# ahcorde/visualSLAM_Android

Measured on AMD Instinct MI355X. Metric: frames/sec (TrackFrame+local BA) on 640×480 synthetic, 1/2/4/8 GPU, higher is better.
Workload: dtype f64

## Files before the change

### visualslam_android_amd/csrc/track.hip

```cpp
#include "vslam_internal.h"
#include "patch_dev.h"
#include "pvs_perm.h"

#define TRK_THREADS 256
#define SORT_CAP 4096
static_assert(SORT_CAP == PVS_SORT_CAP, "a level's list (at most max_points entries) fits the permutation's sort buffer");

template <class T>
DEVFN bool td_project(T& td, int& flags, const double* pos, const Pose& pose, const CamModel& cam, CamProj& pr) {
  flags &= ~TDF_IN_IMAGE;
  double c[3];
  pose_xform(pose, pos, c);
  td.cam[0] = c[0]; td.cam[1] = c[1]; td.cam[2] = c[2];
  if (c[2] < 0.001) return false;
  const double implane[2] = {c[0] / c[2], c[1] / c[2]};
  if (implane[0] * implane[0] + implane[1] * implane[1] > cam.largest_radius * cam.largest_radius) return false;
  pr = cam_project(cam, implane[0], implane[1]);
  td.image[0] = pr.im[0]; td.image[1] = pr.im[1];
  if (pr.invalid) return true;
  if (td.image[0] < 0 || td.image[1] < 0 || td.image[0] > cam.size[0] || td.image[1] > cam.size[1]) return true;
  flags |= TDF_IN_IMAGE;
  return true;
}

// ... 116 lines not shown
  for (int l = 0; l < NLEV; l++) pvs_shuffle_list(pvs_sortbuf(), pvs + l * P, cnt[l], h, l);
}

template <bool SHUFFLE>
__global__ __launch_bounds__(TRK_THREADS) void k_plan(MapDev m, TrackParams tp, int stage) {
  const int s = blockIdx.x;
  TrackerState* st = &m.st[s];
  if (!trk_runs_track_map(st)) return;
  const int P = tp.max_points;
  TrackData* td = m.td + (size_t)s * P;
  const MapPointDev* pts = m.pts + (size_t)s * P;
  int* pvs = m.pvs_list + (size_t)s * NLEV * P;
  int2* slist = m.search_list + (size_t)s * P;
  int* ilist = m.iter_list + (size_t)s * P;
  const int lane = threadIdx.x & 63, wave = threadIdx.x >> 6;
  __shared__ int cnt[NLEV];
  __shared__ int wcnt[TRK_THREADS / 64][NLEV];
  __shared__ int plan[4];
  if (stage == 0) {
    if (threadIdx.x < NLEV) cnt[threadIdx.x] = 0;
    __syncthreads();
    const int n = st->n_points;
    constexpr int PLAN_CH = 16;
    for (int base = 0; base < n; base += PLAN_CH * TRK_THREADS) {
      const int first = base + threadIdx.x * PLAN_CH;
      int lv[PLAN_CH], c[NLEV] = {0, 0, 0, 0};
#pragma unroll
      for (int k = 0; k < PLAN_CH; k++) { const int i = first + k; lv[k] = m.pt_level[(size_t)s * P + (i < n ? i : n - 1)]; if (i >= n) lv[k] = -1; }
#pragma unroll
      for (int k = 0; k < PLAN_CH; k++)
#pragma unroll
        for (int l = 0; l < NLEV; l++) c[l] += lv[k] == l;
      int off[NLEV];
#pragma unroll
      for (int l = 0; l < NLEV; l++) {
        int inc = c[l];
        for (int d = 1; d < 64; d <<= 1) { const int t = __shfl_up(inc, d); if (lane >= d) inc += t; }
        if (lane == 63) wcnt[wave][l] = inc;
        off[l] = inc - c[l];
      }
      __syncthreads();
#pragma unroll
      for (int l = 0; l < NLEV; l++) { off[l] += cnt[l]; for (int w = 0; w < wave; w++) off[l] += wcnt[w][l]; }
#pragma unroll
      for (int k = 0; k < PLAN_CH; k++) {
#pragma unroll
        for (int l = 0; l < NLEV; l++) if (lv[k] == l) pvs[l * P + off[l]++] = first + k;
      }
      __syncthreads();
      if (threadIdx.x < NLEV) { int t = cnt[threadIdx.x]; for (int w = 0; w < TRK_THREADS / 64; w++) t += wcnt[w][threadIdx.x]; cnt[threadIdx.x] = t; }
      __syncthreads();
    }
    if constexpr (SHUFFLE) {
      const unsigned seed = st->pvs_seed;
      if (seed) pvs_shuffle_levels(pvs, P, cnt, seed, st->frame);
    }
    if (threadIdx.x == 0) {
      for (int l = 0; l < NLEV; l++) { st->pvs_count[l] = cnt[l]; st->pvs_head[l] = 0; }
      unsigned nCoarseMax = tp.coarse_max, nCoarseRange = tp.coarse_range;
      st->did_coarse = 0;
      bool bTry = true;
      if (tp.coarse_disabled || st->msd_vel < tp.coarse_min_vel || nCoarseMax == 0) bTry = false;
      if (st->just_recovered) { bTry = true; nCoarseMax *= 2; nCoarseRange *= 2; st->just_recovered = 0; }
      int c3 = 0, c2 = 0;
      const unsigned n3 = cnt[3], n2 = cnt[2];
      if (bTry && n3 + n2 > (unsigned)tp.coarse_min) {
        unsigned take3 = n3 <= nCoarseMax ? n3 : nCoarseMax;
        st->pvs_head[3] = take3;
        c3 = take3;
        if (take3 < nCoarseMax) {
          const unsigned more = nCoarseMax - take3;
          if (n2 <= more) { c3 = 0; c2 = n2; st->pvs_head[2] = n2; }
          else { c2 = more; st->pvs_head[2] = more; }
        }
      }
      plan[0] = c3; plan[1] = c2;
      st->coarse_range = nCoarseRange;
      st->n_coarse = c3 + c2; st->n_search = c3 + c2; st->n_iter = c3 + c2;
    }
    __syncthreads();
    const int c3 = plan[0], c2 = plan[1];
    for (int e = threadIdx.x; e < c3 + c2; e += TRK_THREADS) {
      const int idx = e < c3 ? pvs[3 * P + e] : pvs[2 * P + (e - c3)];
      slist[e] = make_int2(idx, tp.coarse_subpix_its);
      ilist[e] = idx;
    }
  } else {
    __shared__ Pose pose;
    if (threadIdx.x == 0) {
      pose = st->pose_cur;
      const int nit = st->n_iter;
      const int h3 = st->pvs_head[3], n3 = st->pvs_count[3] - h3;
      int nother = (st->pvs_count[2] - st->pvs_head[2]) + st->pvs_count[1] + st->pvs_count[0];
      int nFine = tp.max_patches - (nit + n3);
      if (nFine < 0) nFine = 0;
      if constexpr (SHUFFLE) *pvs_chopped() = nother > nFine && nFine > 0 && st->pvs_seed != 0;
      if (nother > nFine) nother = nFine;
      plan[0] = nit; plan[1] = n3; plan[2] = nother;
      st->fine_range = st->did_coarse ? 5 : 10;
      st->n_l3 = n3; st->n_search = n3 + nother; st->n_iter = nit + n3 + nother;
    }
    __syncthreads();
    const int nit = plan[0], n3 = plan[1], nother = plan[2];
    const int h3 = st->pvs_head[3], h2 = st->pvs_head[2];
    const int r2 = st->pvs_count[2] - h2, r1 = st->pvs_count[1];
    const int did_coarse = st->did_coarse;
    const uint64_t* rest_order = nullptr;
    if constexpr (SHUFFLE) {
      uint64_t* sortbuf = pvs_sortbuf();
      if (*pvs_chopped()) {
        const int nrest = r2 + r1 + st->pvs_count[0];
        pvs_block_fill<TRK_THREADS>(sortbuf, nrest, pvs_frame_hash(st->pvs_seed, st->frame), PVS_LIST_REST, nullptr);
        pvs_block_sort<TRK_THREADS>(sortbuf, nrest);
        rest_order = sortbuf;
      }
    }
    for (int e = threadIdx.x; e < n3 + nother; e += TRK_THREADS) {
      int idx, its;
      if (e < n3) { idx = pvs[3 * P + h3 + e]; its = tp.fine_subpix_its; }
      else {
        int k = e - n3;
        if constexpr (SHUFFLE) if (rest_order) k = (int)(uint32_t)rest_order[k];
        if (k < r2) idx = pvs[2 * P + h2 + k];
        else if (k < r2 + r1) idx = pvs[1 * P + (k - r2)];
        else idx = pvs[0 * P + (k - r2 - r1)];
        its = 0;
      }
      if (e < n3 || did_coarse) td_project_and_derivs(td[idx], m.pt_flags[(size_t)s * P + idx], pts[idx].pos, pose, tp.cam);
      slist[e] = make_int2(idx, its);
      ilist[nit + e] = idx;
    }
  }
}

struct SearchArgs {
  const uint8_t* img[NLEV]; size_t img_sstride[NLEV]; int img_pitch[NLEV];
  const uint32_t* corners[NLEV]; const int* rowlut[NLEV]; const int* ncorners;
  int w[NLEV], h[NLEV], cap[NLEV];
  size_t kf_stride[NLEV];
  int kf_pitch[NLEV];
  int nblk, S;
};


#define TRK_XCDS 8
DEVFN void xcd_stream_block(int nblk, int S, int& s, int& blk) {
  const int i = blockIdx.x, x = i % TRK_XCDS, j = i / TRK_XCDS;
  blk = j % nblk;
  s = (j / nblk) * TRK_XCDS + x;
  if (s >= S) s = -1;
}
static int xcd_grid(int nblk, int S) { return nblk * ((S + TRK_XCDS - 1) / TRK_XCDS) * TRK_XCDS; }

template <int PS, int G>
__global__ __launch_bounds__(64) void k_searchN(MapDev m, TrackParams tp, SearchArgs a, int stage) {
  constexpr int NPIX = PS * PS, HALF = PS / 2, PPW = 64 / G;
  int s, bx;
  xcd_stream_block(a.nblk, a.S, s, bx);
  if (s < 0) return;
  TrackerState* st = &m.st[s];
  if (!trk_runs_track_map(st)) return;
  const int nsearch = st->n_search;
  if (bx * PPW >= nsearch) return;
  const int lane = threadIdx.x, grp = lane / G, sub = lane % G;
  const bool rowact = sub < PS;
  const int e = bx * PPW + grp;
  bool act = e < nsearch;
  const bool lead = sub == 0;
  const int2 ent = act ? m.search_list[(size_t)s * tp.max_points + e] : make_int2(0, 0);
  const int idx = ent.x, nSubPixIts = ent.y;
  const int nRangeL0 = stage == 0 ? st->coarse_range : st->fine_range;
  TrackData& td = m.td[(size_t)s * tp.max_points + idx];
  int& tdlevel = m.pt_level[(size_t)s * tp.max_points + idx];
  int& tdflags = m.pt_flags[(size_t)s * tp.max_points + idx];
  const MapPointDev& p = m.pts[(size_t)s * tp.max_points + idx];
  uint8_t* gtmpl = m.tmpl + ((size_t)s * tp.max_points + idx) * TMPL_PITCH;
  const int level = act ? tdlevel : 0, scale = 1 << level;
  int flags = tdflags;

  double m2[4];
  template_warp_matrix(td.warp_inv, scale, m2);
  const bool refresh = (!(flags & TDF_HAVE_LAST) || warp_moved(m2, td.last_warp)) && act;
  PRow<PS> trow = zero_row<PS>();
  if (rowact) trow = load_row<PS>(gtmpl + sub * PS);
  const int tsum_cached = td.tsum, tsumsq_cached = td.tsumsq;
  int tsum, tsumsq;
  if (__any(refresh)) {
    const int sl = p.src_level;
    const uint8_t* src = m.kf_img[sl] + ((size_t)s * tp.max_keyframes + p.src_kf) * a.kf_stride[sl];
    const int sp = a.kf_pitch[sl], iw = a.w[sl], ih = a.h[sl];
    const TemplateWarp tw = template_warp<PS>(m2, p.irx, p.iry, iw, ih);
    double px = tw.x0, py = tw.y0;
#pragma unroll 1
    for (int i = 0; i < PS - 1; i++) {
      if (i < sub) warp_row_step<PS>(tw, px, py);
    }
    if (refresh) {
      int nOutside = 0, sum = 0, sumsq = 0;
      if (rowact) {
        trow = zero_row<PS>();
#pragma unroll
        for (int j = 0; j < PS; j++) {
          const int v = warp_sample(tw, src, sp, px, py, nOutside);
          warp_pixel_step(tw, px, py);
          trow.w[j >> 2] |= (unsigned)v << (8 * (j & 3));
          sum += v; sumsq += v * v;
        }
        __builtin_memcpy(gtmpl + sub * PS, &trow, PS);
      }
      nOutside = grp_sum<G>(nOutside);
      tsum = grp_sum<G>(sum); tsumsq = grp_sum<G>(sumsq);
      flags = nOutside ? (flags | TDF_TMPL_BAD) : (flags & ~TDF_TMPL_BAD);
      flags |= TDF_HAVE_LAST;
      if (lead) { td.tsum = tsum; td.tsumsq = tsumsq; for (int i = 0; i < 4; i++) td.last_warp[i] = m2[i]; }
    }
  }
  if (!refresh) { tsum = tsum_cached; tsumsq = tsumsq_cached; }
  if (act && (flags & TDF_TMPL_BAD)) {
    if (lead) tdflags = flags & ~(TDF_IN_IMAGE | TDF_FOUND);
    act = false;
  }
  for (int l = 0; l < NLEV; l++) {
    const int c = __popcll(__ballot(act && lead && level == l));
    if (lane == 0 && c) atomicAdd(&st->attempted[l], c);
  }

  const double irx = td.image[0] / scale, iry = td.image[1] / scale;
  const int rows = a.h[level], cols = a.w[level];
  const CoarseWindow cw = coarse_window(irx, iry, nRangeL0, scale, rows);
  int nBestSSD = tp.max_ssd + 1;
  uint32_t bestCorner = 0;
  unsigned nEval = 0;
  const uint32_t* corners = a.corners[level] + (size_t)s * a.cap[level];
  const uint8_t* img = a.img[level] + (size_t)s * a.img_sstride[level];
  const int ip = a.img_pitch[level];
  int i0 = 0, i1 = 0;
  if (act && !cw.empty) {
    const int* lut = a.rowlut[level] + (size_t)s * (rows + 1);
    i0 = lut[cw.top];
    i1 = cw.bottom_plus_one >= rows ? a.ncorners[s * NLEV + level] : lut[cw.bottom_plus_one];
  }
  const double r2max = (double)(cw.range * cw.range);
  constexpr int CPL = 4;
  for (int base = i0; __any(base < i1); base += CPL * G) {
    uint32_t cval[CPL];
    unsigned long long gm = 0;
#pragma unroll
    for (int j = 0; j < CPL; j++) {
      const int ci = base + j * G + sub;
      cval[j] = ci < i1 ? corners[ci] : 0u;
    }
#pragma unroll
    for (int j = 0; j < CPL; j++) {
      const int ci = base + j * G + sub;
      bool ok = false;
      if (ci < i1) {
        const int cx = cval[j] & 0xFFFF, cy = cval[j] >> 16;
        if (!(cx < cw.left || cx > cw.right)) {
          const double dx = irx - cx, dy = iry - cy;
          ok = !(dx * dx + dy * dy > r2max);
        }
      }
      gm |= (unsigned long long)((unsigned)(__ballot(ok) >> (grp * G)) & ((1u << G) - 1u)) << (j * G);
    }
    nEval += __popcll(gm);
    while (__any(gm != 0)) {
      int kk[2]; bool has[2], inside[2]; uint32_t c[2]; PRow<PS> n[2];
#pragma unroll
      for (int u = 0; u < 2; u++) {
        has[u] = gm != 0;
        kk[u] = has[u] ? __ffsll((long long)gm) - 1 : 0;
        gm &= gm - 1;
        const int j = kk[u] / G;
        const uint32_t csel = j == 0 ? cval[0] : (j == 1 ? cval[1] : (j == 2 ? cval[2] : cval[3]));
        c[u] = __shfl(csel, grp * G + (kk[u] % G));
        const int cx = c[u] & 0xFFFF, cy = c[u] >> 16;
        inside[u] = has[u] && cx >= HALF && cy >= HALF && cx < cols - HALF && cy < rows - HALF;
        n[u] = zero_row<PS>();
        if (inside[u] && rowact) n[u] = load_row<PS>(img + (size_t)(cy - HALF + sub) * ip + (cx - HALF));
      }
#pragma unroll
      for (int u = 0; u < 2; u++) {
        int sA, sQ, sX;
        grp_zmssd_sums<PS, G>(n[u], trow, sA, sQ, sX);
        if (has[u]) {
          const int ssd = inside[u] ? zmssd_score<NPIX>(tsum, tsumsq, sA, sQ, sX) : tp.max_ssd + 1;
          if (ssd < nBestSSD) { nBestSSD = ssd; bestCorner = c[u]; }
        }
      }
    }
  }
  flags |= TDF_SEARCHED;
  {
    const int tot = wave_sum(act && lead ? (int)nEval : 0);
    if (lane == 0 && tot) atomicAdd(&st->n_zmssd, (unsigned long long)tot);
  }
  bool found = act && nBestSSD < tp.max_ssd;
  if (act && !found && lead) tdflags = flags & ~TDF_FOUND;
  const uint32_t bc = found ? bestCorner : 0u;
  const double coarse[2] = {level_zero_pos((double)(bc & 0xFFFF), level), level_zero_pos((double)(bc >> 16), level)};
  if (found) flags |= TDF_FOUND;
  const bool dosub = found && nSubPixIts > 0;
  if (found) {
    flags = dosub ? (flags | TDF_SUBPIX) : (flags & ~TDF_SUBPIX);
    if (lead) { tdflags = flags; td.sqrt_inv_noise = 1.0 / scale; td.vfound[0] = coarse[0]; td.vfound[1] = coarse[1]; }
  }
  for (int l = 0; l < NLEV; l++) {
    const int c = __popcll(__ballot(found && !dosub && lead && level == l));
    if (lane == 0 && c) atomicAdd(&st->found[l], c);
  }
}

template <int PS, int G>
DEVFN void subpix_block(const MapDev& m, const TrackParams& tp, const SearchArgs& a, TrackerState* st, int s, int nsub, int blk) {
  constexpr int HALF = PS / 2, PPW = 64 / G, NW = (PS + 3) / 4, Q = PS - 2;
  const int lane = threadIdx.x, grp = lane / G, sub = lane % G;
  const int e = blk * PPW + grp;
  const bool lead = sub == 0;
  const int2 ent = e < nsub ? m.search_list[(size_t)s * tp.max_points + e] : make_int2(0, 0);
  const int idx = ent.x, nSubPixIts = ent.y;
  TrackData& td = m.td[(size_t)s * tp.max_points + idx];
  int& tdlevel = m.pt_level[(size_t)s * tp.max_points + idx];
  int& tdflags = m.pt_flags[(size_t)s * tp.max_points + idx];
  int flags = tdflags;
  const bool dosub = e < nsub && nSubPixIts > 0 && (flags & TDF_FOUND) && (flags & TDF_SUBPIX);
  if (!__any(dosub)) return;
  const int level = dosub ? tdlevel : 0, scale = 1 << level;
  const int rows = a.h[level], cols = a.w[level];
  const uint8_t* img = a.img[level] + (size_t)s * a.img_sstride[level];
  const int ip = a.img_pitch[level];
  PRow<PS> trow = zero_row<PS>(), rup, rdn;
  if (sub < PS) trow = load_row<PS>(m.tmpl + ((size_t)s * tp.max_points + idx) * TMPL_PITCH + sub * PS);
  const bool rowok = sub >= 1 && sub <= Q;
#pragma unroll
  for (int k = 0; k < NW; k++) { rup.w[k] = __shfl(trow.w[k], lane - 1); rdn.w[k] = __shfl(trow.w[k], lane + 1); }
  double gx[Q], gy[Q];
  double h00 = 0, h01 = 0, h02 = 0, h11 = 0, h12 = 0, h22 = 0;
#pragma unroll
  for (int x = 1; x <= Q; x++) {
    gx[x - 1] = 0; gy[x - 1] = 0;
    if (rowok) {
      gx[x - 1] = 0.5 * (row_byte(trow, x + 1) - row_byte(trow, x - 1));
      gy[x - 1] = 0.5 * (row_byte(rdn, x) - row_byte(rup, x));
      h00 += gx[x - 1] * gx[x - 1]; h01 += gx[x - 1] * gy[x - 1]; h02 += gx[x - 1];
      h11 += gy[x - 1] * gy[x - 1]; h12 += gy[x - 1]; h22 += 1.0;
    }
  }
  h00 = grp_sum<G>(h00); h01 = grp_sum<G>(h01); h02 = grp_sum<G>(h02);
  h11 = grp_sum<G>(h11); h12 = grp_sum<G>(h12); h22 = grp_sum<G>(h22);
  const double H[9] = {h00, h01, h02, h01, h11, h12, h02, h12, h22};
  double Hinv[9];
  inv3(H, Hinv);
  double sub0 = td.vfound[0], sub1 = td.vfound[1], meanDiff = 0.0;
  bool running = dosub, converged = false;
  for (int it = 0; __any(running); it++) {
    if (it >= nSubPixIts) running = false;
    double cx = 0, cy = 0;
    if (running) {
      cx = level_n_pos(sub0, level); cy = level_n_pos(sub1, level);
      const int xb = (int)(cx > 0.0 ? cx + 0.5 : cx - 0.5), yb = (int)(cy > 0.0 ? cy + 0.5 : cy - 0.5);
      const int b = HALF + 1;
      if (!(xb >= b && yb >= b && xb < cols - b && yb < rows - b)) running = false;
    }
    double p0[Q], p1[Q], p2[Q];
#pragma unroll
    for (int x = 0; x < Q; x++) { p0[x] = 0; p1[x] = 0; p2[x] = 0; }
    if (running && rowok) {
      const double bx = cx - HALF, by = cy - HALF;
      const double dX = bx - floor(bx), dY = by - floor(by);
      const float fTL = (float)((1.0 - dX) * (1.0 - dY)), fTR = (float)((dX) * (1.0 - dY));
      const float fBL = (float)((1.0 - dX) * (dY)), fBR = (float)((dX) * (dY));
      const uint8_t* r0 = img + (size_t)((int)by + sub) * ip + (int)bx + 1;
      const PRow<PS> q0 = load_row<PS>(r0), q1 = load_row<PS>(r0 + ip);
#pragma unroll
      for (int x = 1; x <= Q; x++) {
        const float fPixel = fTL * row_byte(q0, x - 1) + fTR * row_byte(q0, x) + fBL * row_byte(q1, x - 1) + fBR * row_byte(q1, x);
        const double dDiff = (fPixel - (float)row_byte(trow, x)) + meanDiff;
        p0[x - 1] = dDiff * gx[x - 1]; p1[x - 1] = dDiff * gy[x - 1]; p2[x - 1] = dDiff;
      }
    }
    double a0 = 0, a1 = 0, a2 = 0;
#pragma unroll 1
    for (int y = 1; y <= Q; y++) {
      if (sub == y) {
#pragma unroll
        for (int x = 0; x < Q; x++) { a0 += p0[x]; a1 += p1[x]; a2 += p2[x]; }
      }
      const int src = grp * G + y;
      a0 = __shfl(a0, src); a1 = __shfl(a1, src); a2 = __shfl(a2, src);
    }
    if (running) {
      const double u0 = Hinv[0] * a0 + Hinv[1] * a1 + Hinv[2] * a2;
      const double u1 = Hinv[3] * a0 + Hinv[4] * a1 + Hinv[5] * a2;
      const double u2 = Hinv[6] * a0 + Hinv[7] * a1 + Hinv[8] * a2;
      sub0 -= u0 * scale; sub1 -= u1 * scale; meanDiff -= u2;
      if (u0 * u0 + u1 * u1 < 0.03 * 0.03) { converged = true; running = false; }
    }
  }
  if (dosub && lead) {
    if (!converged) tdflags = flags & ~TDF_FOUND;
    else { td.vfound[0] = sub0; td.vfound[1] = sub1; }
  }
  for (int l = 0; l < NLEV; l++) {
    const int c = __popcll(__ballot(dosub && converged && lead && level == l));
    if (lane == 0 && c) atomicAdd(&st->found[l], c);
  }
}

#define SUBPIX_GRID 16
template <int PS, int G>
__global__ __launch_bounds__(64) void k_subpixN(MapDev m, TrackParams tp, SearchArgs a, int stage) {
  int s, bx;
  xcd_stream_block(a.nblk, a.S, s, bx);
  if (s < 0) return;
  TrackerState* st = &m.st[s];
  if (!trk_runs_track_map(st)) return;
  const int nsub = stage == 0 ? st->n_search : st->n_l3;
  for (int blk = bx; blk * (64 / G) < nsub; blk += a.nblk) subpix_block<PS, G>(m, tp, a, st, s, nsub, blk);
}

#define POSE_THREADS 128
#ifdef VSLAM_BA_PROF
__device__ unsigned long long g_pose_prof[16];
#define POSE_STAMP(id) do { if (blockIdx.x == 0 && threadIdx.x == 0) { const unsigned long long t_ = clock64(); g_pose_prof[id] += t_ - g_pose_prof[15]; g_pose_prof[15] = t_; } } while (0)
#else
#define POSE_STAMP(id) do { } while (0)
#endif
#define POSE_WAVES (POSE_THREADS / 64)
#ifndef POSE_ILP
#define POSE_ILP 2
#endif

struct PoseItem {
  double cam[3], image[2], derivs[4], vfound[2], sqrt_inv_noise;
  int flags, idx;
};
struct PoseWs { double* d; int* i; int P; };

DEVFN void item_load(PoseItem& it, const PoseWs& w, int e) {
  it.flags = w.i[e]; it.idx = w.i[w.P + e];
#pragma unroll
  for (int i = 0; i < 3; i++) it.cam[i] = w.d[(0 + i) * w.P + e];
#pragma unroll
  for (int i = 0; i < 2; i++) { it.image[i] = w.d[(3 + i) * w.P + e]; it.vfound[i] = w.d[(9 + i) * w.P + e]; }
#pragma unroll
  for (int i = 0; i < 4; i++) it.derivs[i] = w.d[(5 + i) * w.P + e];
  it.sqrt_inv_noise = w.d[11 * w.P + e];
}
DEVFN void item_store(const PoseItem& it, const PoseWs& w, int e, bool all) {
#pragma unroll
  for (int i = 0; i < 2; i++) w.d[(3 + i) * w.P + e] = it.image[i];
  if (!all) return;
  w.i[e] = it.flags;
#pragma unroll
  for (int i = 0; i < 3; i++) w.d[(0 + i) * w.P + e] = it.cam[i];
#pragma unroll
  for (int i = 0; i < 4; i++) w.d[(5 + i) * w.P + e] = it.derivs[i];
}

#define POSE_CHUNK 32
#define POSE_ENT 27
#define POSE_GRP 8
static_assert(2 * 2 * POSE_CHUNK * POSE_ENT + 2 * POSE_GRP * POSE_ENT + 64 <= SORT_CAP, "two record buffers (and the chain's two groups of read-ahead) in the sort buffer");
// ... 251 lines not shown
    const bool nonlinear = stage == 0 || iter == 0 || iter == 4 || iter == 9;
    for (int e0 = threadIdx.x; e0 < nf; e0 += POSE_ILP * POSE_THREADS) {
      PoseItem t[POSE_ILP]; double pos[POSE_ILP][3];
#pragma unroll
      for (int u = 0; u < POSE_ILP; u++) {
        const int e = e0 + u * POSE_THREADS;
        item_load(t[u], ws, e < nf ? e : nf - 1);
      }
      if (nonlinear && iter != 0) {
#pragma unroll
        for (int u = 0; u < POSE_ILP; u++)
#pragma unroll
          for (int k = 0; k < 3; k++) pos[u][k] = pts[t[u].idx].pos[k];
      }
#pragma unroll
      for (int u = 0; u < POSE_ILP; u++) {
        const int e = e0 + u * POSE_THREADS;
        if (e >= nf) continue;
        if (iter != 0) {
          if (nonlinear) td_project_and_derivs(t[u], t[u].flags, pos[u], pose, tp.cam);
          else {
            double jac[12], a = 0, b = 0;
            td_calc_jacobian(t[u], jac);
#pragma unroll
            for (int k = 0; k < 6; k++) { a += jac[k] * last_up[k]; b += jac[6 + k] * last_up[k]; }
            t[u].image[0] += a; t[u].image[1] += b;
          }
          item_store(t[u], ws, e, nonlinear);
        }
        const double r0 = (t[u].vfound[0] - t[u].image[0]) * t[u].sqrt_inv_noise;
        const double r1 = (t[u].vfound[1] - t[u].image[1]) * t[u].sqrt_inv_noise;
        sortbuf[e] = r0 * r0 + r1 * r1;
      }
    }
    __syncthreads();
    POSE_STAMP(1);
    const double override_sigma = iter > 5 ? (stage == 0 ? 1.0 : 16.0) : 0.0;
    calc_pose_update(ws, pts, nf, tp, override_sigma, stage == 1 && iter == 9, sortbuf, red, up, hist, sel);
    if (threadIdx.x == 0) pose = pose_mul(se3_exp(up), pose);
    if (threadIdx.x < 6) last_up[threadIdx.x] = up[threadIdx.x];
    __syncthreads();
    POSE_STAMP(7);
  }
  POSE_STAMP(8);
  MeasDev* cm = m.cur_meas + (size_t)s * P;
  if (stage != 0) {
    for (int i = threadIdx.x; i < st->n_points; i += POSE_THREADS) cm[i].valid = 0;
    __syncthreads();
  }
  for (int e0 = threadIdx.x; e0 < nf; e0 += POSE_GB * POSE_THREADS) {
    int idx[POSE_GB], fl[POSE_GB], lv[POSE_GB]; double v[POSE_GB][11];
#pragma unroll
    for (int u = 0; u < POSE_GB; u++) {
      const int e = e0 + u * POSE_THREADS, ec = e < nf ? e : nf - 1;
      idx[u] = ws.i[P + ec]; fl[u] = ws.i[ec];
#pragma unroll
      for (int c = 0; c < 11; c++) v[u][c] = ws.d[c * P + ec];
    }
    if (stage != 0) {
#pragma unroll
      for (int u = 0; u < POSE_GB; u++) lv[u] = m.pt_level[(size_t)s * P + idx[u]];
    }
#pragma unroll
    for (int u = 0; u < POSE_GB; u++) {
      const int e = e0 + u * POSE_THREADS;
      if (e >= nf) continue;
      TrackData& t = td[idx[u]];
      m.pt_flags[(size_t)s * P + idx[u]] = fl[u];
      for (int i = 0; i < 3; i++) t.cam[i] = v[u][i];
      for (int i = 0; i < 2; i++) t.image[i] = v[u][3 + i];
      for (int i = 0; i < 4; i++) t.derivs[i] = v[u][5 + i];
      if (stage != 0) {
        MeasDev mm;
        mm.root[0] = v[u][9]; mm.root[1] = v[u][10];
        mm.valid = 1; mm.level = (signed char)lv[u]; mm.subpix = (fl[u] & TDF_SUBPIX) ? 1 : 0; mm.source = 0 ; mm.pad = 0;
        cm[idx[u]] = mm;
        sortbuf[e] = v[u][2];
      }
    }
  }
  if (stage == 0) {
    if (threadIdx.x == 0) { st->pose_cur = pose; st->did_coarse = 1; }
    return;
  }
  __syncthreads();
  if (threadIdx.x < 2) {
    double a = 0.0;
    const bool sq = threadIdx.x == 1;
    int k = 0;
    for (; k + 8 <= nf; k += 8) {
      double z[8];
#pragma unroll
      for (int u = 0; u < 8; u++) z[u] = sortbuf[k + u];
#pragma unroll
      for (int u = 0; u < 8; u++) a += sq ? z[u] * z[u] : z[u];
    }
    for (; k < nf; k++) { const double z = sortbuf[k]; a += sq ? z * z : z; }
    red[threadIdx.x] = a;
  }
  __syncthreads();
  if (threadIdx.x != 0) return;
  const double dSum = red[0], dSumSq = red[1];
  const int nNum = nf;
  if (nNum > 20) {
    st->depth_mean = dSum / nNum;
    st->depth_sigma = sqrt((dSumSq / nNum) - (st->depth_mean) * (st->depth_mean));
  }
  st->pose_cur = pose; st->pose_final = pose;
  const bool recovered = st->recovered_now != 0;
  st->recovered_now = 0;
  if (!recovered) {
    const Pose nfo = pose_mul(pose, pose_inverse(st->start_pose));
    double motion[6];
    se3_ln(nfo, motion);
    double ss = 0;
    for (int i = 0; i < 6; i++) {
      st->velocity[i] = 0.9 * (0.5 * motion[i] + 0.5 * st->velocity[i]);
      double v = st->velocity[i];
      if (i < 3) v *= 1.0 / st->depth_mean;
      ss += v * v;
    }
    st->msd_vel = sqrt(ss);
  }
  const Pose* kfp = m.kf_pose + (size_t)s * tp.max_keyframes;
  double closest = 9999999999.9;
  for (int k = 0; k < st->n_kf; k++) { const double d = kf_linear_dist(pose, kfp[k]); if (d < closest) closest = d; }
  {
    int ta = 0, tf = 0, la = 0, lf = 0;
    for (int i = 0; i < NLEV; i++) { ta += st->attempted[i]; tf += st->found[i]; if (i >= 2) { la += st->attempted[i]; lf += st->found[i]; } }
    int quality;
    if (tf == 0 || ta == 0) quality = 0;
    else {
      const double dTotal = (double)tf / ta;
      const double dLarge = la > 10 ? (double)lf / la : dTotal;
      if (dTotal > 0.3) quality = 2; else if (dLarge < 0.13) quality = 0; else quality = 1;
    }
    if (quality == 1 && closest > tp.wiggle_scale * 10.0) quality = 0;
    if (quality == 0) st->lost_frames++; else st->lost_frames = 0;
    st->quality = quality;
  }
  if (!recovered) {
    double dDist = closest;
    dDist *= (1.0 / st->depth_mean);
    const bool need = dDist > tp.max_kf_dist_wiggle_mult * st->wiggle_depth_norm;
    if (st->quality == 2 && need && st->frame - st->last_kf_dropped > tp.min_frames_between_kf && st->n_kf < tp.max_keyframes) {
      st->kf_pending = 1;
      st->last_kf_dropped = st->frame;
    }
  }
  POSE_STAMP(9);
}

#ifdef VSLAM_BA_PROF
extern "C" int vslam_debug_pose_prof(unsigned long long* out16, int reset) {
  HIPCHK(hipDeviceSynchronize());
  HIPCHK(hipMemcpyFromSymbol(out16, HIP_SYMBOL(g_pose_prof), sizeof(unsigned long long) * 16));
  if (reset) { unsigned long long z[16] = {0}; HIPCHK(hipMemcpyToSymbol(HIP_SYMBOL(g_pose_prof), z, sizeof(z))); }
  return VSLAM_OK;
}
#endif

#define TALLOC(ptr, count) do { int _r = dev_alloc(sys, &(ptr), (count)); if (_r) return _r; } while (0)

int trk_alloc(vslam_system* sys) {
  const vslam_params& p = sys->p;
  const size_t S = sys->S, P = p.max_points, K = p.max_keyframes;
  if (P > SORT_CAP) { vslam_set_error("max_points %d exceeds %d", (int)P, SORT_CAP); return VSLAM_E_INVALID; }
  MapDev& m = sys->map;
  TALLOC(m.pts, S * P); TALLOC(m.td, S * P); TALLOC(m.tmpl, S * P * TMPL_PITCH);
  TALLOC(m.kf_meas, S * K * P); TALLOC(m.cur_meas, S * P);
  TALLOC(m.kf_pose, S * K); TALLOC(m.kf_fixed, S * K); TALLOC(m.kf_depth, S * K * 2);
  for (int l = 0; l < NLEV; l++) TALLOC(m.kf_img[l], S * K * (size_t)sys->geom[l].pitch * sys->geom[l].h);
  TALLOC(m.st, S); TALLOC(m.pvs_list, S * NLEV * P); TALLOC(m.search_list, S * P); TALLOC(m.iter_list, S * P); TALLOC(m.pt_level, S * P); TALLOC(m.pt_flags, S * P);
  TALLOC(m.pose_ws, S * POSE_WS_COMPS * P); TALLOC(m.pose_wsi, S * 2 * P);
  trk_fill_params(p, sys->tp);
  return VSLAM_OK;
}

void cam_fill(CamModel& c, const double cam5[5], double width, double height, int quirks) {
  c.size[0] = width; c.size[1] = height;
  c.focal[0] = c.size[0] * cam5[0]; c.focal[1] = c.size[1] * cam5[1];
  c.center[0] = c.size[0] * cam5[2] - 0.5; c.center[1] = c.size[1] * cam5[3] - 0.5;
  c.w = cam5[4];
  double one_over_2tan = 0;
  if (c.w != 0.0) { c.two_tan = 2.0 * vlm::vtan(c.w / 2.0); one_over_2tan = 1.0 / c.two_tan; c.winv = 1.0 / c.w; c.distortion_enabled = 1.0; }
  else { c.winv = 0; c.two_tan = 0; c.distortion_enabled = 0; }
  double v2[2];
  if (quirks & VSLAM_Q_CAM_INT_RADIUS) {
    int m1 = (int)cam5[2], m2 = (int)(1.0 - cam5[2]);
    v2[0] = (m1 > m2 ? m1 : m2) / cam5[0];
    m1 = (int)cam5[3]; m2 = (int)(1.0 - cam5[3]);
    v2[1] = (m1 > m2 ? m1 : m2) / cam5[1];
  } else {
    v2[0] = (cam5[2] > 1.0 - cam5[2] ? cam5[2] : 1.0 - cam5[2]) / cam5[0];
    v2[1] = (cam5[3] > 1.0 - cam5[3] ? cam5[3] : 1.0 - cam5[3]) / cam5[1];
  }
  const double rr = sqrt(v2[0] * v2[0] + v2[1] * v2[1]);
  c.largest_radius = c.w == 0.0 ? rr : vlm::vtan(rr * c.w) * one_over_2tan;
  c.max_r = 1.5 * c.largest_radius;
}

void trk_fill_params(const vslam_params& p, TrackParams& t) {
  cam_fill(t.cam, p.cam, p.width, p.height, p.quirks);
  t.P = p.patch_size; t.max_ssd = 500 * p.patch_size * p.patch_size;
  t.max_patches = p.max_patches_per_frame; t.coarse_min = p.coarse_min; t.coarse_max = p.coarse_max; t.coarse_range = p.coarse_range;
  t.coarse_subpix_its = p.coarse_subpix_its; t.coarse_disabled = p.coarse_disabled; t.fine_subpix_its = p.fine_subpix_its;
  t.coarse_min_vel = p.coarse_min_vel; t.wls_prior = p.wls_prior;
  t.min_frames_between_kf = p.min_frames_between_kf; t.max_kf_dist_wiggle_mult = p.max_kf_dist_wiggle_mult; t.wiggle_scale = p.wiggle_scale;
  t.ba_max_iterations = p.ba_max_iterations; t.ba_convergence_limit = p.ba_convergence_limit;
  t.ba_min_sigma2 = p.ba_min_tukey_sigma * p.ba_min_tukey_sigma; t.ba_window = p.ba_window; t.ba_min_keyframes = p.ba_min_keyframes;
  t.quirks = p.quirks; t.max_points = p.max_points; t.max_keyframes = p.max_keyframes; t.ba_delay = p.ba_delay_frames;
  t.ba_batch = p.ba_batch_frames > 1 ? p.ba_batch_frames : 1;
  t.ba_sum_order = p.ba_sum_order ? 1 : 0;
  t.grow_map = p.grow_map;
  t.idle = p.idle_iterations != 0; t.fq_cap = 8192;
  {
    double a[2], b[2];
    cam_unproject(t.cam, t.cam.size[0] / 2, t.cam.size[1] / 2, a);
    cam_unproject(t.cam, t.cam.size[0] / 2 + 1, t.cam.size[1] / 2 + 1, b);
    const double d0 = a[0] - b[0], d1 = a[1] - b[1];
    t.one_pixel_dist = sqrt(d0 * d0 + d1 * d1) / sqrt(2.0);
  }
  const int kcap_max[NLEV] = {16384, 8192, 4096, 2048};
  for (int l = 0; l < NLEV; l++) t.kcap[l] = p.max_corners[l] < kcap_max[l] ? p.max_corners[l] : kcap_max[l];

}

static void trk_search_args(vslam_system* sys, SearchArgs& a) {
  for (int l = 0; l < NLEV; l++) {
    a.img[l] = sys->fr.img[l]; a.img_sstride[l] = sys->fr.img_sstride[l]; a.img_pitch[l] = sys->fr.img_pitch[l];
    a.corners[l] = sys->fr.corners[l]; a.rowlut[l] = sys->fr.rowlut[l];
    a.w[l] = sys->geom[l].w; a.h[l] = sys->geom[l].h; a.cap[l] = sys->geom[l].cap;
    a.kf_pitch[l] = sys->geom[l].pitch; a.kf_stride[l] = (size_t)sys->geom[l].pitch * sys->geom[l].h;
  }
  a.ncorners = sys->fr.ncorners;
}

typedef void (*PlanKernel)(MapDev, TrackParams, int);
static PlanKernel plan_kernel(const vslam_system* sys) { return sys->p.pvs_shuffle_seed ? k_plan<true> : k_plan<false>; }

int trk_search_stage(vslam_system* sys, int stage) {
  const int S = sys->S, P = sys->p.max_points;
  MapDev& m = sys->map;
  const TrackParams& tp = sys->tp;
  SearchArgs a;
  trk_search_args(sys, a);
  a.S = S; a.nblk = 1;
  if (stage == 0) {
    prof_mark(sys, PROF_PVS);
    hipLaunchKernelGGL(k_motion, dim3((S + 63) / 64), dim3(64), 0, sys->stream, m, S, sys->p.use_sbi ? (const double*)sys->fr.sbi_rot : (const double*)nullptr);
    hipLaunchKernelGGL(k_pvs, dim3((P + TRK_THREADS - 1) / TRK_THREADS, S), dim3(TRK_THREADS), 0, sys->stream, m, tp);
    prof_mark(sys, PROF_PLAN_COARSE);
    hipLaunchKernelGGL(plan_kernel(sys), dim3(S), dim3(TRK_THREADS), 0, sys->stream, m, tp, 0);
    prof_mark(sys, PROF_SEARCH_COARSE);
    if (!tp.coarse_disabled || sys->p.relocalise) {
      const int nc = 2 * tp.coarse_max;
      if (tp.P == 8) {
        a.nblk = (nc + 7) / 8; hipLaunchKernelGGL((k_searchN<8, 8>), dim3(xcd_grid(a.nblk, S)), dim3(64), 0, sys->stream, m, tp, a, 0);
        if (tp.coarse_subpix_its > 0) { a.nblk = SUBPIX_GRID; hipLaunchKernelGGL((k_subpixN<8, 8>), dim3(xcd_grid(a.nblk, S)), dim3(64), 0, sys->stream, m, tp, a, 0); }
      } else {
        a.nblk = (nc + 3) / 4; hipLaunchKernelGGL((k_searchN<11, 16>), dim3(xcd_grid(a.nblk, S)), dim3(64), 0, sys->stream, m, tp, a, 0);
        if (tp.coarse_subpix_its > 0) { a.nblk = SUBPIX_GRID; hipLaunchKernelGGL((k_subpixN<11, 16>), dim3(xcd_grid(a.nblk, S)), dim3(64), 0, sys->stream, m, tp, a, 0); }
      }
    }
    prof_mark(sys, PROF_POSE_COARSE);
  } else {
    const int maxSearch = tp.max_patches + 2 * tp.coarse_max < P ? tp.max_patches + 2 * tp.coarse_max : P;
    prof_mark(sys, PROF_PLAN_FINE);
    hipLaunchKernelGGL(plan_kernel(sys), dim3(S), dim3(TRK_THREADS), 0, sys->stream, m, tp, 1);
    prof_mark(sys, PROF_SEARCH_FINE);
    if (tp.P == 8) {
      a.nblk = (maxSearch + 7) / 8; hipLaunchKernelGGL((k_searchN<8, 8>), dim3(xcd_grid(a.nblk, S)), dim3(64), 0, sys->stream, m, tp, a, 1);
      if (tp.fine_subpix_its > 0) { a.nblk = SUBPIX_GRID; hipLaunchKernelGGL((k_subpixN<8, 8>), dim3(xcd_grid(a.nblk, S)), dim3(64), 0, sys->stream, m, tp, a, 1); }
    } else {
      a.nblk = (maxSearch + 3) / 4; hipLaunchKernelGGL((k_searchN<11, 16>), dim3(xcd_grid(a.nblk, S)), dim3(64), 0, sys->stream, m, tp, a, 1);
      if (tp.fine_subpix_its > 0) { a.nblk = SUBPIX_GRID; hipLaunchKernelGGL((k_subpixN<11, 16>), dim3(xcd_grid(a.nblk, S)), dim3(64), 0, sys->stream, m, tp, a, 1); }
    }
    prof_mark(sys, PROF_POSE_FINE);
  }
  HIPCHK(hipGetLastError());
  return VSLAM_OK;
}

int trk_pose_stage(vslam_system* sys, int stage) {
  if (stage == 0 && sys->tp.coarse_disabled && !sys->p.relocalise) return VSLAM_OK;
  hipLaunchKernelGGL(k_pose, dim3(sys->S), dim3(POSE_THREADS), 0, sys->stream, sys->map, sys->tp, stage);
  HIPCHK(hipGetLastError());
  return VSLAM_OK;
}

int trk_track_map(vslam_system* sys) {
  int r = trk_search_stage(sys, 0);
  if (!r) r = trk_pose_stage(sys, 0);
  if (!r) r = trk_search_stage(sys, 1);
  if (!r) r = trk_pose_stage(sys, 1);
  return r;
}

__global__ void k_set_pvs_seed(MapDev m, int S, int stream, unsigned seed) {
  const int s = blockIdx.x * blockDim.x + threadIdx.x;
  if (s >= S || (stream >= 0 && s != stream)) return;
  m.st[s].pvs_seed = seed;
}

extern "C" int vslam_set_pvs_seed(vslam_system* sys, int stream, unsigned seed) {
  if (!sys || stream >= sys->S) { vslam_set_error("set_pvs_seed: bad argument"); return VSLAM_E_INVALID; }
// ... 50 lines not shown
```

Measured before the change: 481,300.

## Widen corner-search batches, stage candidates in LDS, process K candidates per trip

```diff
diff --git a/visualslam_android_amd/csrc/track.hip b/visualslam_android_amd/csrc/track.hip
--- a/visualslam_android_amd/csrc/track.hip
+++ b/visualslam_android_amd/csrc/track.hip
@@ -292,6 +292,48 @@
 }
 static int xcd_grid(int nblk, int S) { return nblk * ((S + TRK_XCDS - 1) / TRK_XCDS) * TRK_XCDS; }
 
+#ifndef SEARCH_N
+#define SEARCH_N 128
+#endif
+#ifndef SEARCH_K
+#define SEARCH_K 4
+#endif
+#ifdef VSLAM_BA_PROF
+#define SEARCH_PROF_SLOTS 64
+__device__ unsigned long long g_search_prof[2][SEARCH_PROF_SLOTS];
+enum { SP_ENTRY, SP_TEMPLATE, SP_LUT, SP_FILTER, SP_ZMSSD, SP_WRITE, SP_PHASES };
+#define SEARCH_PROF(...) __VA_ARGS__
+#define SEARCH_PROF_BEGIN() const bool sp_on = (blockIdx.x / TRK_XCDS) % 7 == 0; unsigned long long sp_ph[SP_PHASES] = {0, 0, 0, 0, 0, 0}, sp_t0 = clock64(); \
+  int sp_ftrips = 0, sp_ztrips = 0, sp_ncorners = 0; bool sp_refresh = false
+#define SEARCH_STAMP(id) do { if (sp_on) { const unsigned long long t_ = clock64(); sp_ph[id] += t_ - sp_t0; sp_t0 = t_; } } while (0)
+#define SEARCH_PROF_END() do { if (sp_on) search_prof_flush(g_search_prof[stage], sp_ph, sp_ftrips, sp_ztrips, sp_refresh, e < nsearch && lead, sp_ncorners, (int)nEval); } while (0)
+DEVFN void search_prof_flush(unsigned long long* g, const unsigned long long* ph, int ftrips, int ztrips, bool refresh, bool patch, int ncorners, int nsurv) {
+  if (threadIdx.x == 0) {
+    for (int i = 0; i < SP_PHASES; i++) atomicAdd(&g[i], ph[i]);
+    atomicAdd(&g[6], 1ull); atomicAdd(&g[7], refresh ? 1ull : 0ull); atomicAdd(&g[8], (unsigned long long)ftrips); atomicAdd(&g[9], (unsigned long long)ztrips);
+    atomicAdd(&g[34 + (ftrips < 5 ? ftrips : 5)], 1ull); atomicAdd(&g[40 + (ztrips < 9 ? ztrips : 9)], 1ull);
+  }
+  if (patch) {
+    atomicAdd(&g[10], (unsigned long long)((nsurv + SEARCH_K - 1) / SEARCH_K)); atomicAdd(&g[11], 1ull);
+    atomicAdd(&g[12], (unsigned long long)nsurv); atomicAdd(&g[13], (unsigned long long)ncorners);
+    const int cb = ncorners == 0 ? 0 : ncorners <= 64 ? 1 + (ncorners - 1) / 16 : ncorners <= 128 ? 5 + (ncorners - 65) / 32 : 7;
+    const int sb = nsurv <= 4 ? nsurv : nsurv <= 16 ? 5 + (nsurv - 5) / 4 : 8;
+    atomicAdd(&g[16 + cb], 1ull); atomicAdd(&g[24 + sb], 1ull);
+  }
+}
+#else
+#define SEARCH_PROF(...)
+#define SEARCH_PROF_BEGIN() do { } while (0)
+#define SEARCH_STAMP(id) do { } while (0)
+#define SEARCH_PROF_END() do { } while (0)
+#endif
+
+DEVFN void wave_lds_sync() {
+  __builtin_amdgcn_fence(__ATOMIC_RELEASE, "wavefront");
+  __builtin_amdgcn_wave_barrier();
+  __builtin_amdgcn_fence(__ATOMIC_ACQUIRE, "wavefront");
+}
+
 template <int PS, int G>
 __global__ __launch_bounds__(64) void k_searchN(MapDev m, TrackParams tp, SearchArgs a, int stage) {
   constexpr int NPIX = PS * PS, HALF = PS / 2, PPW = 64 / G;
@@ -307,6 +349,7 @@
   const int e = bx * PPW + grp;
   bool act = e < nsearch;
   const bool lead = sub == 0;
+  SEARCH_PROF_BEGIN();
   const int2 ent = act ? m.search_list[(size_t)s * tp.max_points + e] : make_int2(0, 0);
   const int idx = ent.x, nSubPixIts = ent.y;
   const int nRangeL0 = stage == 0 ? st->coarse_range : st->fine_range;
@@ -317,14 +360,22 @@
   uint8_t* gtmpl = m.tmpl + ((size_t)s * tp.max_points + idx) * TMPL_PITCH;
   const int level = act ? tdlevel : 0, scale = 1 << level;
   int flags = tdflags;
-
-  double m2[4];
-  template_warp_matrix(td.warp_inv, scale, m2);
-  const bool refresh = (!(flags & TDF_HAVE_LAST) || warp_moved(m2, td.last_warp)) && act;
+  const double td_image[2] = {td.image[0], td.image[1]};
+  const double td_warp_inv[4] = {td.warp_inv[0], td.warp_inv[1], td.warp_inv[2], td.warp_inv[3]};
+  const double td_last_warp[4] = {td.last_warp[0], td.last_warp[1], td.last_warp[2], td.last_warp[3]};
+  const int tsum_cached = td.tsum, tsumsq_cached = td.tsumsq;
   PRow<PS> trow = zero_row<PS>();
   if (rowact) trow = load_row<PS>(gtmpl + sub * PS);
-  const int tsum_cached = td.tsum, tsumsq_cached = td.tsumsq;
+    struct PatchRec { double irx, iry; int left, right; unsigned range; int flags, level, subpix_its, idx, pad; };
+  __shared__ PatchRec wrec[PPW];
+  if (lead) { wrec[grp].irx = td_image[0] / scale; wrec[grp].iry = td_image[1] / scale; }
+  SEARCH_STAMP(SP_ENTRY);
+
+  double m2[4];
+  template_warp_matrix(td_warp_inv, scale, m2);
+  const bool refresh = (!(flags & TDF_HAVE_LAST) || warp_moved(m2, td_last_warp)) && act;
   int tsum, tsumsq;
+  SEARCH_PROF(sp_refresh = __any(refresh) != 0;)
   if (__any(refresh)) {
     const int sl = p.src_level;
     const uint8_t* src = m.kf_img[sl] + ((size_t)s * tp.max_keyframes + p.src_kf) * a.kf_stride[sl];
@@ -360,67 +411,95 @@
     if (lead) tdflags = flags & ~(TDF_IN_IMAGE | TDF_FOUND);
     act = false;
   }
-  for (int l = 0; l < NLEV; l++) {
-    const int c = __popcll(__ballot(act && lead && level == l));
-    if (lane == 0 && c) atomicAdd(&st->attempted[l], c);
-  }
-
-  const double irx = td.image[0] / scale, iry = td.image[1] / scale;
+  const bool attempted = act;
+  SEARCH_STAMP(SP_TEMPLATE);
+
+  wave_lds_sync();
+  const double irx = wrec[grp].irx, iry = wrec[grp].iry;
   const int rows = a.h[level], cols = a.w[level];
   const CoarseWindow cw = coarse_window(irx, iry, nRangeL0, scale, rows);
+  int i0 = 0, i1 = 0;
+  if (act && !cw.empty) {
+    const int* lut = a.rowlut[level] + (size_t)s * (rows + 1);
+    const int below = cw.bottom_plus_one >= rows ? rows : cw.bottom_plus_one;
+    const int n_all = a.ncorners[s * NLEV + level], lut_top = lut[cw.top], lut_below = lut[below];
+    i0 = lut_top;
+    i1 = cw.bottom_plus_one >= rows ? n_all : lut_below;
+  }
   int nBestSSD = tp.max_ssd + 1;
   uint32_t bestCorner = 0;
   unsigned nEval = 0;
   const uint32_t* corners = a.corners[level] + (size_t)s * a.cap[level];
   const uint8_t* img = a.img[level] + (size_t)s * a.img_sstride[level];
   const int ip = a.img_pitch[level];
-  int i0 = 0, i1 = 0;
-  if (act && !cw.empty) {
-    const int* lut = a.rowlut[level] + (size_t)s * (rows + 1);
-    i0 = lut[cw.top];
-    i1 = cw.bottom_plus_one >= rows ? a.ncorners[s * NLEV + level] : lut[cw.bottom_plus_one];
-  }
-  const double r2max = (double)(cw.range * cw.range);
-  constexpr int CPL = 4;
+  SEARCH_PROF(sp_ncorners = i1 - i0;)
+  constexpr int CPL = SEARCH_N / G < 4 ? 4 : SEARCH_N / G, K = SEARCH_K, NM = (CPL * G + 63) / 64;
+  static_assert(64 % G == 0, "a lane group's bits of one ballot lie in one mask word");
+  constexpr int CSTRIDE = CPL * G + G;
+  __shared__ uint32_t ctrip[PPW * CSTRIDE];
+  uint32_t* const gtrip = ctrip + grp * CSTRIDE;
+  if (lead) {
+    wrec[grp].left = cw.left; wrec[grp].right = cw.right; wrec[grp].range = cw.range;
+    wrec[grp].flags = flags; wrec[grp].level = level; wrec[grp].subpix_its = nSubPixIts; wrec[grp].idx = idx;
+  }
+  wave_lds_sync();
   for (int base = i0; __any(base < i1); base += CPL * G) {
     uint32_t cval[CPL];
-    unsigned long long gm = 0;
+    unsigned long long gm[NM];
+#pragma unroll
+    for (int w = 0; w < NM; w++) gm[w] = 0;
+    const double wx = wrec[grp].irx, wy = wrec[grp].iry, r2max = (double)(wrec[grp].range * wrec[grp].range);
+    const int wleft = wrec[grp].left, wright = wrec[grp].right;
 #pragma unroll
     for (int j = 0; j < CPL; j++) {
       const int ci = base + j * G + sub;
       cval[j] = ci < i1 ? corners[ci] : 0u;
     }
+    SEARCH_STAMP(SP_LUT);
 #pragma unroll
     for (int j = 0; j < CPL; j++) {
       const int ci = base + j * G + sub;
       bool ok = false;
       if (ci < i1) {
         const int cx = cval[j] & 0xFFFF, cy = cval[j] >> 16;
-        if (!(cx < cw.left || cx > cw.right)) {
-          const double dx = irx - cx, dy = iry - cy;
+        if (!(cx < wleft || cx > wright)) {
+          const double dx = wx - cx, dy = wy - cy;
           ok = !(dx * dx + dy * dy > r2max);
         }
       }
-      gm |= (unsigned long long)((unsigned)(__ballot(ok) >> (grp * G)) & ((1u << G) - 1u)) << (j * G);
-    }
-    nEval += __popcll(gm);
-    while (__any(gm != 0)) {
-      int kk[2]; bool has[2], inside[2]; uint32_t c[2]; PRow<PS> n[2];
-#pragma unroll
-      for (int u = 0; u < 2; u++) {
-        has[u] = gm != 0;
-        kk[u] = has[u] ? __ffsll((long long)gm) - 1 : 0;
-        gm &= gm - 1;
-        const int j = kk[u] / G;
-        const uint32_t csel = j == 0 ? cval[0] : (j == 1 ? cval[1] : (j == 2 ? cval[2] : cval[3]));
-        c[u] = __shfl(csel, grp * G + (kk[u] % G));
+      gm[j * G / 64] |= (unsigned long long)((unsigned)(__ballot(ok) >> (grp * G)) & ((1u << G) - 1u)) << (j * G % 64);
+      gtrip[j * G + sub] = cval[j];
+    }
+    wave_lds_sync();
+    unsigned long long left = 0;
+#pragma unroll
+    for (int w = 0; w < NM; w++) { nEval += __popcll(gm[w]); left |= gm[w]; }
+    SEARCH_PROF(sp_ftrips++;)
+    SEARCH_STAMP(SP_FILTER);
+    while (__any(left != 0)) {
+      bool has[K], inside[K]; uint32_t c[K]; PRow<PS> n[K];
+#pragma unroll
+      for (int u = 0; u < K; u++) {
+        has[u] = left != 0;
+        int kk = 0;
+        bool taken = false;
+        left = 0;
+#pragma unroll
+        for (int w = 0; w < NM; w++) {
+          const bool here = !taken && gm[w] != 0;
+          if (here) { kk = 64 * w + __ffsll((long long)gm[w]) - 1; gm[w] &= gm[w] - 1; }
+          taken = taken || here;
+          left |= gm[w];
+        }
+        c[u] = gtrip[kk];
         const int cx = c[u] & 0xFFFF, cy = c[u] >> 16;
         inside[u] = has[u] && cx >= HALF && cy >= HALF && cx < cols - HALF && cy < rows - HALF;
         n[u] = zero_row<PS>();
         if (inside[u] && rowact) n[u] = load_row<PS>(img + (size_t)(cy - HALF + sub) * ip + (cx - HALF));
       }
 #pragma unroll
-      for (int u = 0; u < 2; u++) {
+      for (int u = 0; u < K; u++) {
+        if (u >= 2 && !__any(has[u])) break;
         int sA, sQ, sX;
         grp_zmssd_sums<PS, G>(n[u], trow, sA, sQ, sX);
         if (has[u]) {
@@ -428,27 +507,37 @@
           if (ssd < nBestSSD) { nBestSSD = ssd; bestCorner = c[u]; }
         }
       }
-    }
-  }
-  flags |= TDF_SEARCHED;
+      SEARCH_PROF(sp_ztrips++;)
+      SEARCH_STAMP(SP_ZMSSD);
+    }
+    wave_lds_sync();
+  }
+  SEARCH_STAMP(SP_LUT);
   {
     const int tot = wave_sum(act && lead ? (int)nEval : 0);
     if (lane == 0 && tot) atomicAdd(&st->n_zmssd, (unsigned long long)tot);
   }
-  bool found = act && nBestSSD < tp.max_ssd;
-  if (act && !found && lead) tdflags = flags & ~TDF_FOUND;
+  const int wlevel = wrec[grp].level, wits = wrec[grp].subpix_its;
+  int wflags = wrec[grp].flags | TDF_SEARCHED;
+  const size_t gi = (size_t)s * tp.max_points + wrec[grp].idx;
+  const bool found = act && nBestSSD < tp.max_ssd;
+  if (act && !found && lead) m.pt_flags[gi] = wflags & ~TDF_FOUND;
   const uint32_t bc = found ? bestCorner : 0u;
-  const double coarse[2] = {level_zero_pos((double)(bc & 0xFFFF), level), level_zero_pos((double)(bc >> 16), level)};
-  if (found) flags |= TDF_FOUND;
-  const bool dosub = found && nSubPixIts > 0;
+  const double coarse[2] = {level_zero_pos((double)(bc & 0xFFFF), wlevel), level_zero_pos((double)(bc >> 16), wlevel)};
+  if (found) wflags |= TDF_FOUND;
+  const bool dosub = found && wits > 0;
   if (found) {
-    flags = dosub ? (flags | TDF_SUBPIX) : (flags & ~TDF_SUBPIX);
-    if (lead) { tdflags = flags; td.sqrt_inv_noise = 1.0 / scale; td.vfound[0] = coarse[0]; td.vfound[1] = coarse[1]; }
+    wflags = dosub ? (wflags | TDF_SUBPIX) : (wflags & ~TDF_SUBPIX);
+    if (lead) { TrackData& tdw = m.td[gi]; m.pt_flags[gi] = wflags; tdw.sqrt_inv_noise = 1.0 / (1 << wlevel); tdw.vfound[0] = coarse[0]; tdw.vfound[1] = coarse[1]; }
   }
   for (int l = 0; l < NLEV; l++) {
-    const int c = __popcll(__ballot(found && !dosub && lead && level == l));
+    const int ca = __popcll(__ballot(attempted && lead && wlevel == l));
+    if (lane == 0 && ca) atomicAdd(&st->attempted[l], ca);
+    const int c = __popcll(__ballot(found && !dosub && lead && wlevel == l));
     if (lane == 0 && c) atomicAdd(&st->found[l], c);
   }
+  SEARCH_STAMP(SP_WRITE);
+  SEARCH_PROF_END();
 }
 
 template <int PS, int G>
@@ -1006,6 +1095,13 @@
 }
 
 #ifdef VSLAM_BA_PROF
+extern "C" int vslam_debug_search_prof(unsigned long long* out, int reset) {
+  HIPCHK(hipDeviceSynchronize());
+  HIPCHK(hipMemcpyFromSymbol(out, HIP_SYMBOL(g_search_prof), sizeof(unsigned long long) * 2 * SEARCH_PROF_SLOTS));
+  if (reset) { unsigned long long z[2 * SEARCH_PROF_SLOTS] = {0}; HIPCHK(hipMemcpyToSymbol(HIP_SYMBOL(g_search_prof), z, sizeof(z))); }
+  out[15] = SEARCH_N; out[SEARCH_PROF_SLOTS + 15] = SEARCH_K;
+  return VSLAM_OK;
+}
 extern "C" int vslam_debug_pose_prof(unsigned long long* out16, int reset) {
   HIPCHK(hipDeviceSynchronize());
   HIPCHK(hipMemcpyFromSymbol(out16, HIP_SYMBOL(g_pose_prof), sizeof(unsigned long long) * 16));
```

Result: faster. 492,500, median of 6 (+2.3%).
